# zellerlab/GECCO

Measured on AMD Instinct MI355X. Metric: genes/sec CRF decode (windowed fwd-bwd marginals + Viterbi), higher is better.
Workload: dtype f64

## Files before the change

gecco_amd/csrc/crf_scan.hpp:

```cpp
#pragma once
#include "crf_device.hpp"

namespace gecco {
namespace {

constexpr int kScanThreads = 256;

struct MapOp {
    static __device__ __forceinline__ uint32_t identity() { return 2u; }
    static __device__ __forceinline__ uint32_t combine(uint32_t a, uint32_t b) {
        return ((a >> (b & 1u)) & 1u) | (((a >> ((b >> 1) & 1u)) & 1u) << 1);
    }
};


template <int CTRL, int RM>
__device__ __forceinline__ double dpp_f64(double old, double src) {
    int lo = __builtin_amdgcn_update_dpp(__double2loint(old), __double2loint(src), CTRL, RM, 0xF, false);
    int hi = __builtin_amdgcn_update_dpp(__double2hiint(old), __double2hiint(src), CTRL, RM, 0xF, false);
    return __hiloint2double(hi, lo);
}
template <int CTRL, int RM>
__device__ __forceinline__ VE dpp_elem(const VE &old, const VE &s) {
    return VE{dpp_f64<CTRL, RM>(old.a00, s.a00), dpp_f64<CTRL, RM>(old.a01, s.a01), dpp_f64<CTRL, RM>(old.a10, s.a10),
              dpp_f64<CTRL, RM>(old.a11, s.a11), dpp_f64<CTRL, RM>(old.rs, s.rs)};
}
template <int CTRL, int RM>
__device__ __forceinline__ FE dpp_elem(const FE &old, const FE &s) {
    return FE{dpp_f64<CTRL, RM>(old.a00, s.a00), dpp_f64<CTRL, RM>(old.a01, s.a01), dpp_f64<CTRL, RM>(old.a10, s.a10),
              dpp_f64<CTRL, RM>(old.a11, s.a11), dpp_f64<CTRL, RM>(old.ex, s.ex),   dpp_f64<CTRL, RM>(old.ms, s.ms),
              dpp_f64<CTRL, RM>(old.rs, s.rs)};
}
template <int CTRL, int RM>
__device__ __forceinline__ CE dpp_elem(const CE &old, const CE &s) {
    return CE{dpp_f64<CTRL, RM>(old.a, s.a), dpp_f64<CTRL, RM>(old.L, s.L), dpp_f64<CTRL, RM>(old.H, s.H)};
}
template <int CTRL, int RM>
__device__ __forceinline__ SegE dpp_elem(const SegE &old, const SegE &s) {
    auto mv = [](uint32_t o, uint32_t v) { return uint32_t(__builtin_amdgcn_update_dpp(int(o), int(v), CTRL, RM, 0xF, false)); };
    return SegE{mv(old.map, s.map), mv(old.ng0, s.ng0), mv(old.ng1, s.ng1), mv(old.ann, s.ann)};
}
struct F4 {
    double a00, a01, a10, a11;
};
template <int CTRL, int RM>
__device__ __forceinline__ F4 dpp_elem(const F4 &old, const F4 &s) {
    return F4{dpp_f64<CTRL, RM>(old.a00, s.a00), dpp_f64<CTRL, RM>(old.a01, s.a01), dpp_f64<CTRL, RM>(old.a10, s.a10),
              dpp_f64<CTRL, RM>(old.a11, s.a11)};
}
struct U2 {
    uint32_t x, y;
};
template <int CTRL, int RM>
__device__ __forceinline__ U2 dpp_elem(const U2 &old, const U2 &s) {
    auto mv = [](uint32_t o, uint32_t v) { return uint32_t(__builtin_amdgcn_update_dpp(int(o), int(v), CTRL, RM, 0xF, false)); };
    return U2{mv(old.x, s.x), mv(old.y, s.y)};
}
struct AddOp {
    static __device__ __forceinline__ U2 identity() { return U2{0u, 0u}; }
    static __device__ __forceinline__ U2 combine(const U2 &a, const U2 &b) { return U2{a.x + b.x, a.y + b.y}; }
};
template <int CTRL, int RM>
__device__ __forceinline__ uint32_t dpp_elem(const uint32_t &old, const uint32_t &s) {
    return uint32_t(__builtin_amdgcn_update_dpp(int(old), int(s), CTRL, RM, 0xF, false));
}

template <class Op, bool REV, class E>
__device__ __forceinline__ E comb(const E &earlier_lane, const E &later_lane) {
    return REV ? Op::combine(later_lane, earlier_lane) : Op::combine(earlier_lane, later_lane);
}
template <class Op, bool REV, class E>
__device__ __forceinline__ E wave_scan_inclusive(E v) {
    const E id = Op::identity();
    v = comb<Op, REV>(dpp_elem<0x111, 0xF>(id, v), v);
    v = comb<Op, REV>(dpp_elem<0x112, 0xF>(id, v), v);
    v = comb<Op, REV>(dpp_elem<0x114, 0xF>(id, v), v);
    v = comb<Op, REV>(dpp_elem<0x118, 0xF>(id, v), v);
    v = comb<Op, REV>(dpp_elem<0x142, 0xA>(id, v), v);
    v = comb<Op, REV>(dpp_elem<0x143, 0xC>(id, v), v);
    return v;
}
template <int CTRL>
__device__ __forceinline__ double dpp_f64_z(double src) {
    int lo = __builtin_amdgcn_update_dpp(0, __double2loint(src), CTRL, 0xF, 0xF, true);
    int hi = __builtin_amdgcn_update_dpp(0, __double2hiint(src), CTRL, 0xF, 0xF, true);
    return __hiloint2double(hi, lo);
}
template <class Op>
__device__ __forceinline__ CE wave_scan_inclusive_masked(CE v) {
    const uint32_t lane = __builtin_amdgcn_mbcnt_hi(~0u, __builtin_amdgcn_mbcnt_lo(~0u, 0u));
    const uint32_t col = lane & 15u;
#define GECCO_MASKED_STEP(CTRL, COND)                                                  \
    {                                                                                  \
        CE t{dpp_f64_z<CTRL>(v.a), dpp_f64_z<CTRL>(v.L), dpp_f64_z<CTRL>(v.H)};         \
        if (COND) Op::combine_into(t, v);                                              \
    }
    GECCO_MASKED_STEP(0x111, col >= 1u)
    GECCO_MASKED_STEP(0x112, col >= 2u)
    GECCO_MASKED_STEP(0x114, col >= 4u)
    GECCO_MASKED_STEP(0x118, col >= 8u)
    GECCO_MASKED_STEP(0x142, (lane & 16u) != 0u)
    GECCO_MASKED_STEP(0x143, lane >= 32u)
#undef GECCO_MASKED_STEP
    return v;
}
template <class E>
__device__ __forceinline__ E wave_shift_up(const E &id, const E &v) {
    return dpp_elem<0x138, 0xF>(id, v);
}
template <class Op, bool REV, class E, int NTH = kScanThreads, bool MASKED = false, bool LAST_USE = false>
__device__ __forceinline__ E block_scan_exclusive(const E &mine, E *lds_totals , E *total) {
    const int lane = threadIdx.x & 63, wave = __builtin_amdgcn_readfirstlane(int(threadIdx.x >> 6));
    const E id = Op::identity();
    E incl;
    if constexpr (MASKED) {
        static_assert(!REV, "the masked scan runs in lane order");
        incl = wave_scan_inclusive_masked<Op>(mine);
    } else {
        incl = wave_scan_inclusive<Op, REV>(mine);
    }
    if (lane == 63) lds_totals[wave] = incl;
    E excl = wave_shift_up(id, incl);
    __syncthreads();
    E pre = id, all = id;
#pragma unroll
    for (int w = 0; w < NTH / 64; ++w) {
        const E t = lds_totals[w];
        if (w < wave) pre = comb<Op, REV>(pre, t);
        if (total) all = comb<Op, REV>(all, t);
    }
    if (!LAST_USE) __syncthreads();
    if (total) *total = all;
    return comb<Op, REV>(pre, excl);
}

template <class Op, int NTH = kScanThreads>
__device__ __forceinline__ uint32_t block_scan_exclusive_back(uint32_t mine, uint32_t *lds_totals , uint32_t *total,
                                                              int *vote = nullptr) {
    const int lane = threadIdx.x & 63, wave = __builtin_amdgcn_readfirstlane(int(threadIdx.x >> 6));
    const uint32_t id = Op::identity();
    const int mirror = (63 - lane) << 2;
    const uint32_t m = uint32_t(__builtin_amdgcn_ds_bpermute(mirror, int(mine)));
    const uint32_t incl = wave_scan_inclusive<Op, true>(m);
    if (lane == 63) lds_totals[wave] = incl;
    const uint32_t excl = wave_shift_up(id, incl);
    if (vote) *vote = __syncthreads_or(*vote);
    else __syncthreads();
    uint32_t pre = id, all = id;
#pragma unroll
    for (int w = NTH / 64 - 1; w >= 0; --w) {
        const uint32_t t = lds_totals[w];
        if (w > wave) pre = comb<Op, true>(pre, t);
        all = comb<Op, true>(all, t);
    }
    *total = all;
    return uint32_t(__builtin_amdgcn_ds_bpermute(mirror, int(comb<Op, true>(pre, excl))));
}

}
}
```

gecco_amd/csrc/crf_vd_short.hpp:

```cpp
#pragma once

#include "crf_device.hpp"
#include "crf_scan.hpp"

namespace gecco {
namespace {

constexpr int kT = 256;
constexpr int kGPL = kSeqGenesPerLane;
constexpr int kBlockGenes = kT * kGPL;
static_assert(kBlockGenes == kSeqBlockGenes, "host tables assume this block size");

__device__ __forceinline__ double vd_max(double a, double b) {
    double r;
    asm("v_max_f64 %0, %1, %2" : "=v"(r) : "v"(a), "v"(b));
    return r;
}
__device__ __forceinline__ double vd_min(double a, double b) {
    double r;
    asm("v_min_f64 %0, %1, %2" : "=v"(r) : "v"(a), "v"(b));
    return r;
}
__device__ __forceinline__ double vd_max_s(double a, double bound) {
    double r;
    asm("v_max_f64 %0, %1, %2" : "=v"(r) : "v"(a), "s"(bound));
    return r;
}
__device__ __forceinline__ double vd_min_s(double a, double bound) {
    double r;
    asm("v_min_f64 %0, %1, %2" : "=v"(r) : "v"(a), "s"(bound));
    return r;
}
__device__ __forceinline__ void vd_shift_in_gt(uint32_t &acc, double x, double bound) {
    asm("v_cmp_lt_f64 vcc, %2, %1\n\tv_addc_co_u32 %0, vcc, %0, %0, vcc" : "+v"(acc) : "v"(x), "s"(bound) : "vcc");
}
struct COp {
    static __device__ __forceinline__ CE identity() { return CE{0.0, -__builtin_huge_val(), __builtin_huge_val()}; }
    static __device__ __forceinline__ CE combine(const CE &a, const CE &b) {
        return CE{a.a + b.a, vd_min(vd_max(a.L + b.a, b.L), b.H), vd_min(vd_max(a.H + b.a, b.L), b.H)};
    }
    static __device__ __forceinline__ void combine_into(CE &t, CE &v) {
        asm volatile(
            "v_add_f64 %[tl], %[tl], %[a]\n\t"
            "v_add_f64 %[th], %[th], %[a]\n\t"
            "v_add_f64 %[a], %[ta], %[a]\n\t"
            "v_max_f64 %[tl], %[tl], %[L]\n\t"
            "v_max_f64 %[th], %[th], %[L]\n\t"
            "v_min_f64 %[L], %[tl], %[H]\n\t"
            "v_min_f64 %[H], %[th], %[H]"
            : [a] "+v"(v.a), [L] "+v"(v.L), [H] "+v"(v.H), [tl] "+v"(t.L), [th] "+v"(t.H)
            : [ta] "v"(t.a));
    }
};

__device__ __forceinline__ double vd_bound(const SeqArgs &A, double nnz, double n) { return nnz * A.v_wmax2 + (n + 2.0) * A.v_tmax; }
constexpr double kVdEps = 2.220446049250313e-16;
__device__ __forceinline__ double vd_margin(double r, double ulpM) { return (4.0 * r + 4.0) * ulpM; }

constexpr int kFixChunk = 1024;
struct FixStage {
    double2 st[kFixChunk];
    uint32_t bpw[kFixChunk / 16];
};
__device__ __forceinline__ void exact_states(const SeqArgs &A, int g0, int m, FixStage &fx, int first_lane) {
    const int nl = kT - first_lane, me = int(threadIdx.x) - first_lane;
    if (me < 0) return;
    for (int base = me; base < m; base += 4 * nl) {
        int lo[4], hi[4];
        double s0[4], s1[4];
        int longest = 0;
#pragma unroll
        for (int u = 0; u < 4; ++u) {
            const int i = base + u * nl;
            lo[u] = hi[u] = 0;
            if (i < m) {
                lo[u] = A.csr_gene_ptr[g0 + i];
                hi[u] = A.csr_gene_ptr[g0 + i + 1];
            }
            s0[u] = s1[u] = 0.0;
        }
#pragma unroll
        for (int u = 0; u < 4; ++u) longest = max(longest, hi[u] - lo[u]);
        for (int k = 0; k < longest; ++k) {
            int a[4];
#pragma unroll
            for (int u = 0; u < 4; ++u) a[u] = lo[u] + k < hi[u] ? A.csr_attr_id[lo[u] + k] : -1;
            double2 w[4];
#pragma unroll
            for (int u = 0; u < 4; ++u) w[u] = unsigned(a[u]) < unsigned(A.csr_n_attrs) ? A.csr_wtab01[a[u]] : make_double2(0.0, 0.0);
#pragma unroll
            for (int u = 0; u < 4; ++u) {
                s0[u] += w[u].x;
                s1[u] += w[u].y;
            }
        }
#pragma unroll
        for (int u = 0; u < 4; ++u) {
            const int i = base + u * nl;
            if (i < m) fx.st[i] = make_double2(s0[u], s1[u]);
        }
    }
}
__device__ __forceinline__ void exact_walk(const SeqArgs &A, FixStage &fx, int m, bool first, double &d0, double &d1) {
    int i = 0;
    if (first) {
        d0 = fx.st[0].x;
        d1 = fx.st[0].y;
        i = 1;
    }
    auto step = [&](const double2 s) {
        const double a0 = d0 + A.t00, b0 = d1 + A.t10;
        const double a1 = d0 + A.t01, b1 = d1 + A.t11;
        d0 = fmax(a0, b0) + s.x;
        d1 = fmax(a1, b1) + s.y;
    };
    for (; i < m && (i & 7); ++i) {
        step(fx.st[i]);
        fx.st[i] = make_double2(d0, d1);
    }
    for (; i + 8 <= m; i += 8) {
        double2 sv[8];
#pragma unroll
        for (int u = 0; u < 8; ++u) sv[u] = fx.st[i + u];
#pragma unroll
        for (int u = 0; u < 8; ++u) {
            step(sv[u]);
            fx.st[i + u] = make_double2(d0, d1);
        }
    }
    for (; i < m; ++i) {
        step(fx.st[i]);
        fx.st[i] = make_double2(d0, d1);
    }
}
__device__ __forceinline__ void exact_backpointers(const SeqArgs &A, FixStage &fx, int m, bool first, double e0, double e1) {
    for (int w = threadIdx.x; 16 * w < m; w += kT) {
        uint32_t word = 0;
        for (int i = max(16 * w, first ? 1 : 0); i < min(16 * w + 16, m); ++i) {
            const double p0 = i ? fx.st[i - 1].x : e0, p1 = i ? fx.st[i - 1].y : e1;
            const uint32_t arg0 = (p0 + A.t00) < (p1 + A.t10) ? 1u : 0u, arg1 = (p0 + A.t01) < (p1 + A.t11) ? 1u : 0u;
            word |= (arg0 | (arg1 << 1)) << (2 * (i & 15));
        }
        fx.bpw[w] = word;
    }
}
__device__ __forceinline__ uint32_t *exact_bp_words(const SeqArgs &A, int gs) { return reinterpret_cast<uint32_t *>(A.alpha) + size_t(gs); }
__device__ __forceinline__ uint32_t *exact_end_labels(const SeqArgs &A, int gs) {
    return reinterpret_cast<uint32_t *>(A.alpha) + size_t(A.n_genes) + size_t(gs);
}
__device__ __forceinline__ void exact_backtrack(const SeqArgs &A, int gs, int ge, double d0, double d1) {
    const int n = ge - gs, nw = (n + 15) / 16;
    uint32_t *bpc = exact_bp_words(A, gs), *endl = exact_end_labels(A, gs);
    auto word_map = [&](uint32_t bits, int w, uint32_t y) {
        const int hi = min(16 * w + 15, n - 1), lo = max(16 * w, 1);
        for (int t = hi; t >= lo; --t) y = (bits >> (2 * (t & 15) + y)) & 1u;
        return y;
    };
    for (int w = threadIdx.x; w < nw; w += kT) {
        const uint32_t bits = bpc[w];
        endl[w] = word_map(bits, w, 0) | (word_map(bits, w, 1) << 1);
    }
    __syncthreads();
    if (threadIdx.x == 0) {
        uint32_t y = d0 < d1 ? 1u : 0u;
        for (int w = nw - 1; w >= 0; --w) {
            const uint32_t mp = endl[w];
            endl[w] = y;
            y = (mp >> y) & 1u;
        }
    }
    __syncthreads();
    for (int w = threadIdx.x; w < nw; w += kT) {
        const uint32_t bits = bpc[w];
        uint32_t y = endl[w];
        const int hi = min(16 * w + 15, n - 1), lo = 16 * w;
        for (int t = hi; t >= lo; --t) {
            A.y[gs + t] = int8_t(y);
            if (t >= 1) y = (bits >> (2 * (t & 15) + y)) & 1u;
        }
    }
    __syncthreads();
}

__device__ __forceinline__ void exact_delta_contig(const SeqArgs &A, int gs, int ge, FixStage &fx) {
    uint32_t *bpc = exact_bp_words(A, gs);
    double d0 = 0.0, d1 = 0.0;
    for (int cb = gs; cb < ge; cb += kFixChunk) {
        const int m = min(kFixChunk, ge - cb);
        const double e0 = d0, e1 = d1;
        exact_states(A, cb, m, fx, 0);
        __syncthreads();
        if (threadIdx.x == 0) exact_walk(A, fx, m, cb == gs, d0, d1);
        __syncthreads();
        d0 = fx.st[m - 1].x;
        d1 = fx.st[m - 1].y;
        exact_backpointers(A, fx, m, cb == gs, e0, e1);
        __syncthreads();
        for (int i = threadIdx.x; i < (m + 15) / 16; i += kT) bpc[(cb - gs) / 16 + i] = fx.bpw[i];
        __syncthreads();
    }
    exact_backtrack(A, gs, ge, d0, d1);
}

constexpr double kVdPad = 1e30;

struct VdShortSmem {
    double st[kT * (kGPL + 1)];
    uint32_t mark[kBlockGenes / 32];
    int c_end;
    CE tot[kT / 64];
    uint32_t mtot[kT / 64];
};
static_assert(sizeof(VdShortSmem) <= 20480, "eight workgroups per CU");
__device__ __forceinline__ void load_short(const double *__restrict__ v, int g0, int n, VdShortSmem &stg, double (&x)[kGPL]) {
    const int base = int(threadIdx.x) * kGPL;
    const double *vp = v + g0;
#pragma unroll
    for (int k = 0; k < kGPL; ++k) x[k] = vp[max(min(base + k, n - 1), 0)];
    double *row = stg.st + threadIdx.x * (kGPL + 1);
#pragma unroll
    for (int k = 0; k < kGPL; ++k) {
        x[k] = base + k < n ? x[k] : kVdPad;
        row[k] = x[k];
    }
}

__device__ __forceinline__ uint32_t wave_or_u32(uint32_t v) {
    v |= uint32_t(__builtin_amdgcn_update_dpp(0, int(v), 0x111, 0xF, 0xF, true));
    v |= uint32_t(__builtin_amdgcn_update_dpp(0, int(v), 0x112, 0xF, 0xF, true));
    v |= uint32_t(__builtin_amdgcn_update_dpp(0, int(v), 0x114, 0xF, 0xF, true));
    v |= uint32_t(__builtin_amdgcn_update_dpp(0, int(v), 0x118, 0xF, 0xF, true));
    v |= uint32_t(__builtin_amdgcn_update_dpp(0, int(v), 0x142, 0xA, 0xF, true));
    v |= uint32_t(__builtin_amdgcn_update_dpp(0, int(v), 0x143, 0xC, 0xF, true));
    return uint32_t(__builtin_amdgcn_readlane(int(v), 63));
}

__device__ __forceinline__ void vd_short_block(const SeqArgs &A, const int blk, VdShortSmem &stg) {
    CE *lds = stg.tot;
    uint32_t *ldsm = stg.mtot;
    const int slot = threadIdx.x;
    const int g0 = __builtin_amdgcn_readfirstlane(A.cblk[blk]), n = __builtin_amdgcn_readfirstlane(A.cblk[blk + 1]) - g0;
    const uint32_t bits = A.lane_bits[blk * kT + slot];
    const uint32_t first = bits & 0xffu, last = bits >> 8;
    const uint32_t wave_bits = wave_or_u32(bits);
    double x[kGPL];
    load_short(A.dstate, g0, n, stg, x);
    const int cnt = min(kGPL, n - slot * kGPL);
    const double *row = stg.st + slot * (kGPL + 1);
    CE P = COp::identity();
#pragma unroll
    for (int k = 0; k < kGPL; ++k) {
        const double dvk = x[k];
        const bool fst = (first >> k) & 1u;
        const double c = A.v_k + dvk;
        const double l2 = vd_min_s(vd_max_s(P.L, A.v_lo), A.v_hi) + c, h2 = vd_min_s(vd_max_s(P.H, A.v_lo), A.v_hi) + c;
        P.a += c;
        P.L = l2;
        P.H = h2;
        if ((wave_bits >> k) & 1u) {
            asm volatile("" ::: "memory");
            P.L = fst ? dvk : l2;
            P.H = fst ? dvk : h2;
        }
    }
    const CE M = block_scan_exclusive<COp, false, CE, kScanThreads, true, true>(P, lds, static_cast<CE *>(nullptr));
    double ulpM = 0.0, margin = 1e-6 * fmax(1.0, fmax(fabs(A.v_lo), fabs(A.v_hi)));
    if (A.csr_gene_ptr) {
        ulpM = vd_bound(A, double(A.csr_gene_ptr[g0 + n] - A.csr_gene_ptr[g0]), double(n)) * kVdEps;
        margin = vd_margin(double(n), ulpM);
    }
    ulpM = __hiloint2double(__builtin_amdgcn_readfirstlane(__double2hiint(ulpM)), __builtin_amdgcn_readfirstlane(__double2loint(ulpM)));
    margin = __hiloint2double(__builtin_amdgcn_readfirstlane(__double2hiint(margin)), __builtin_amdgcn_readfirstlane(__double2loint(margin)));
    uint32_t maps = 0, lane_map;
    bool sensitive = false;
    {
        double Dq = M.L;
#pragma unroll
        for (int k = 0; k < kGPL; ++k) {
            const double dvk = row[k];
            const double stepped = vd_min_s(vd_max_s(Dq, A.v_lo), A.v_hi) + (A.v_k + dvk);
            Dq = stepped;
            if ((wave_bits >> k) & 1u) {
                asm volatile("" ::: "memory");
                Dq = ((first >> k) & 1u) ? dvk : stepped;
            }
            vd_shift_in_gt(maps, Dq, A.v_lo);
            vd_shift_in_gt(maps, Dq, A.v_hi);
            bool sens = fabs(Dq - A.v_hi) <= margin || fabs(Dq - A.v_lo) <= margin;
            if ((wave_bits >> (8 + k)) & 1u) {
                asm volatile("" ::: "memory");
                const bool lst = (last >> k) & 1u;
                maps = lst ? ((maps & ~3u) | (Dq > 0.0 ? 3u : 0u)) : maps;
                sens = lst ? fabs(Dq) <= margin : sens;
            }
            sensitive |= sens;
        }
    }
    auto label_map = [&]() {
        uint32_t y0 = 0u, y1 = 1u;
#pragma unroll
        for (int k = kGPL - 1; k >= 0; --k) {
            y0 = __builtin_amdgcn_ubfe(maps, uint32_t(2 * (kGPL - 1 - k)) | y0, 1u);
            y1 = __builtin_amdgcn_ubfe(maps, uint32_t(2 * (kGPL - 1 - k)) | y1, 1u);
        }
        return y0 | (y1 << 1);
    };
    const bool lane_sensitive = sensitive && A.v_exact;
    int vote = lane_sensitive ? 1 : 0;
    uint32_t mtotal;
    lane_map = label_map();
    uint32_t lab = block_scan_exclusive_back<MapOp>(lane_map, ldsm, &mtotal, &vote) & 1u;
    const bool wg_sensitive = vote != 0;
    if (wg_sensitive) {
        double Dq = M.L;
        uint64_t sat = 0;
#pragma unroll
        for (int k = 0; k < kGPL; ++k) {
            if (k < cnt) {
                const double dvk = row[k];
            Dq = ((first >> k) & 1u) ? dvk : fmin(fmax(Dq, A.v_lo), A.v_hi) + (A.v_k + dvk);
                const uint64_t c = Dq >= A.v_hi + margin ? 1u : (Dq <= A.v_lo - margin ? 2u : 0u);
                sat |= c << (8 * k);
            }
        }
        *reinterpret_cast<uint64_t *>(&stg.st[slot * (kGPL + 1) + kGPL]) = sat;
        __syncthreads();
    } else {
        sensitive = false;
    }
    bool lane_flagged = false;
    if (sensitive && cnt > 0) {
        double D = 0.0;
        int r = 0;
        auto certain = [&](double x) { return x >= A.v_hi + margin || x <= A.v_lo - margin; };
        if (!(first & 1u)) {
            const int t0 = slot * kGPL;
            int p = t0 - 1;
            auto dval = [&](int t) { return stg.st[(t / kGPL) * (kGPL + 1) + t % kGPL]; };
            for (;; --p) {
                if (A.flags[g0 + p] & 1u) {
                    D = dval(p);
                    r = 0;
                    break;
                }
                const uint32_t c = reinterpret_cast<const uint8_t *>(&stg.st[((p - 1) / kGPL) * (kGPL + 1) + kGPL])[(p - 1) % kGPL];
                if (c) {
                    D = (c == 1u ? A.v_hi : A.v_lo) + (A.v_k + dval(p));
                    r = 1;
                    break;
                }
            }
            for (int t = p + 1; t < t0; ++t) {
                r = certain(D) ? 1 : r + 1;
                D = fmin(fmax(D, A.v_lo), A.v_hi) + (A.v_k + dval(t));
            }
        }
        maps = 0;
#pragma unroll
        for (int k = 0; k < kGPL; ++k) {
            if (k < cnt) {
                const double dvk = row[k];
                const bool fst = (first >> k) & 1u;
                r = fst ? 0 : (certain(D) ? 1 : r + 1);
                D = fst ? dvk : fmin(fmax(D, A.v_lo), A.v_hi) + (A.v_k + dvk);
                const bool lst = (last >> k) & 1u;
                const double thi = lst ? 0.0 : A.v_hi, tlo = lst ? 0.0 : A.v_lo;
                maps |= ((D > thi ? 1u : 0u) | (D > tlo ? 2u : 0u)) << (2 * (kGPL - 1 - k));
                const double mr = vd_margin(double(r), ulpM);
                lane_flagged |= fabs(D - thi) <= mr || fabs(D - tlo) <= mr;
            }
        }
        if (A.vd_stats) {
            atomicAdd(A.vd_stats + 0, 1u);
            if (lane_flagged) atomicAdd(A.vd_stats + 1, 1u);
        }
    }
    bool wg_flagged = false;
    if (wg_sensitive) {
        wg_flagged = __syncthreads_or(lane_flagged ? 1 : 0);
        lane_map = label_map();
        lab = block_scan_exclusive_back<MapOp>(lane_map, ldsm, &mtotal) & 1u;
    }
    uint64_t packed = 0;
#pragma unroll
    for (int k = kGPL - 1; k >= 0; --k) {
        lab = __builtin_amdgcn_ubfe(maps, uint32_t(2 * (kGPL - 1 - k)) | lab, 1u);
        packed |= uint64_t(lab) << (8 * k);
    }
    {
        struct __attribute__((packed)) Bytes8 {
            uint64_t v;
        };
        int8_t *yp = A.y + g0 + slot * kGPL;
        if (cnt >= kGPL) {
            reinterpret_cast<Bytes8 *>(yp)->v = packed;
        } else {
            for (int k = 0; k < cnt; ++k) yp[k] = int8_t(packed >> (8 * k));
        }
    }
    if (wg_flagged && A.csr_gene_ptr) {
        uint32_t *mark = stg.mark;
        int *c_end = &stg.c_end;
        __syncthreads();
        if (slot < kBlockGenes / 32) mark[slot] = 0;
        __syncthreads();
        if (lane_flagged) {
            int prev = -1;
            for (int k = 0; k < cnt; ++k) {
                int t = slot * kGPL + k;
                while (!(A.flags[g0 + t] & 1u)) --t;
                if (t != prev) atomicOr(&mark[t >> 5], 1u << (t & 31));
                prev = t;
            }
        }
        __syncthreads();
        FixStage &st2 = *reinterpret_cast<FixStage *>(stg.st);
        static_assert(sizeof(stg.st) >= sizeof(FixStage), "exact pass: LDS for one chunk of state scores");
        for (int wi = 0; wi < kBlockGenes / 32; ++wi) {
            uint32_t bits = mark[wi];
            while (bits) {
                const int cs = wi * 32 + __builtin_ctz(bits);
                bits &= bits - 1;
                if (slot == 0) *c_end = n;
                __syncthreads();
                for (int i = cs + slot; i < n; i += kT)
                    if (A.flags[g0 + i] & 2u) {
                        atomicMin(c_end, i + 1);
                        break;
                    }
                __syncthreads();
                const int ce = *c_end;
                __syncthreads();
                if (slot == 0 && A.vd_stats) {
                    atomicAdd(A.vd_stats + 2, 1u);
                    atomicAdd(A.vd_stats + 3, uint32_t(ce - cs));
                }
                exact_delta_contig(A, g0 + cs, g0 + ce, st2);
            }
        }
    }
}

}
}
```

Measured before the change: 73.35 billion.

## Replace clamp scan with short saturation-based propagation and LDS ballot votes

Replaces the full block-wide masked scan of clamp-affine elements with a short local propagation that starts from lanes whose clamp interval has collapsed (L==H). Each lane inherits its neighbour's value for up to a few DPP steps, and the full scan runs only when some wave cannot resolve its inputs that way. It also replaces __syncthreads_or with wave ballots posted to LDS, adds a fast unclamped load path for full waves, and computes sensitivity through one min-abs distance. This cuts scan work and barrier cost in the common saturated case, but adds a fallback branch, extra LDS state and more intricate correctness conditions.

```diff
diff --git a/gecco_amd/csrc/crf_scan.hpp b/gecco_amd/csrc/crf_scan.hpp
--- a/gecco_amd/csrc/crf_scan.hpp
+++ b/gecco_amd/csrc/crf_scan.hpp
@@ -134,9 +134,23 @@
     return comb<Op, REV>(pre, excl);
 }
 
+template <int NTH = kScanThreads>
+__device__ __forceinline__ void block_or_post(bool mine, uint32_t *lds_votes ) {
+    const int wave = __builtin_amdgcn_readfirstlane(int(threadIdx.x >> 6));
+    const uint32_t any = __builtin_amdgcn_ballot_w64(mine) != 0 ? 1u : 0u;
+    if ((threadIdx.x & 63) == 63) lds_votes[wave] = any;
+}
+template <int NTH = kScanThreads>
+__device__ __forceinline__ bool block_or_read(const uint32_t *lds_votes ) {
+    uint32_t any = 0;
+#pragma unroll
+    for (int w = 0; w < NTH / 64; ++w) any |= lds_votes[w];
+    return __builtin_amdgcn_readfirstlane(int(any)) != 0;
+}
+
 template <class Op, int NTH = kScanThreads>
 __device__ __forceinline__ uint32_t block_scan_exclusive_back(uint32_t mine, uint32_t *lds_totals , uint32_t *total,
-                                                              int *vote = nullptr) {
+                                                              int *vote = nullptr, uint32_t *lds_votes  = nullptr) {
     const int lane = threadIdx.x & 63, wave = __builtin_amdgcn_readfirstlane(int(threadIdx.x >> 6));
     const uint32_t id = Op::identity();
     const int mirror = (63 - lane) << 2;
@@ -144,8 +158,9 @@
     const uint32_t incl = wave_scan_inclusive<Op, true>(m);
     if (lane == 63) lds_totals[wave] = incl;
     const uint32_t excl = wave_shift_up(id, incl);
-    if (vote) *vote = __syncthreads_or(*vote);
-    else __syncthreads();
+    if (vote) block_or_post<NTH>(*vote != 0, lds_votes);
+    __syncthreads();
+    if (vote) *vote = block_or_read<NTH>(lds_votes) ? 1 : 0;
     uint32_t pre = id, all = id;
 #pragma unroll
     for (int w = NTH / 64 - 1; w >= 0; --w) {
diff --git a/gecco_amd/csrc/crf_vd_short.hpp b/gecco_amd/csrc/crf_vd_short.hpp
--- a/gecco_amd/csrc/crf_vd_short.hpp
+++ b/gecco_amd/csrc/crf_vd_short.hpp
@@ -19,6 +19,11 @@
 __device__ __forceinline__ double vd_min(double a, double b) {
     double r;
     asm("v_min_f64 %0, %1, %2" : "=v"(r) : "v"(a), "v"(b));
+    return r;
+}
+__device__ __forceinline__ double vd_min_abs(double a, double b) {
+    double r;
+    asm("v_min_f64 %0, |%1|, |%2|" : "=v"(r) : "v"(a), "v"(b));
     return r;
 }
 __device__ __forceinline__ double vd_max_s(double a, double bound) {
@@ -210,14 +215,25 @@
     int c_end;
     CE tot[kT / 64];
     uint32_t mtot[kT / 64];
+    double pv[kT / 64];
+    uint32_t pbad[kT / 64];
+    uint32_t vote[kT / 64];
 };
 static_assert(sizeof(VdShortSmem) <= 20480, "eight workgroups per CU");
 __device__ __forceinline__ void load_short(const double *__restrict__ v, int g0, int n, VdShortSmem &stg, double (&x)[kGPL]) {
     const int base = int(threadIdx.x) * kGPL;
     const double *vp = v + g0;
+    double *row = stg.st + threadIdx.x * (kGPL + 1);
+    const int wave_end = (__builtin_amdgcn_readfirstlane(int(threadIdx.x >> 6)) + 1) * 64 * kGPL;
+    if (wave_end <= n) {
+#pragma unroll
+        for (int k = 0; k < kGPL; ++k) x[k] = vp[base + k];
+#pragma unroll
+        for (int k = 0; k < kGPL; ++k) row[k] = x[k];
+        return;
+    }
 #pragma unroll
     for (int k = 0; k < kGPL; ++k) x[k] = vp[max(min(base + k, n - 1), 0)];
-    double *row = stg.st + threadIdx.x * (kGPL + 1);
 #pragma unroll
     for (int k = 0; k < kGPL; ++k) {
         x[k] = base + k < n ? x[k] : kVdPad;
@@ -233,6 +249,20 @@
     v |= uint32_t(__builtin_amdgcn_update_dpp(0, int(v), 0x142, 0xA, 0xF, true));
     v |= uint32_t(__builtin_amdgcn_update_dpp(0, int(v), 0x143, 0xC, 0xF, true));
     return uint32_t(__builtin_amdgcn_readlane(int(v), 63));
+}
+
+constexpr int kVdRun = 6;
+__device__ __forceinline__ void vd_apply(const CE &P, double in, double &v) {
+    asm volatile("v_add_f64 %0, %1, %2\n\tv_max_f64 %0, %0, %3\n\tv_min_f64 %0, %0, %4" : "+v"(v) : "v"(in), "v"(P.a), "v"(P.L), "v"(P.H));
+}
+__device__ __forceinline__ void vd_propagate(const CE &P, double &v, uint64_t &known) {
+    for (int it = 0; it < kVdRun; ++it) {
+        const uint64_t todo = (known << 1) & ~known;
+        if (!todo) break;
+        const double in = dpp_f64_z<0x138>(v);
+        if (__builtin_amdgcn_inverse_ballot_w64(todo)) vd_apply(P, in, v);
+        known |= todo;
+    }
 }
 
 __device__ __forceinline__ void vd_short_block(const SeqArgs &A, const int blk, VdShortSmem &stg) {
@@ -263,7 +293,29 @@
             P.H = fst ? dvk : h2;
         }
     }
-    const CE M = block_scan_exclusive<COp, false, CE, kScanThreads, true, true>(P, lds, static_cast<CE *>(nullptr));
+    double Din;
+    {
+        const int wave = __builtin_amdgcn_readfirstlane(int(threadIdx.x >> 6));
+        double v = P.L;
+        uint64_t known = __builtin_amdgcn_ballot_w64(P.L == P.H);
+        vd_propagate(P, v, known);
+        const bool wave_bad = (known | (known - 1)) != ~uint64_t(0) || !(known & (wave ? (uint64_t(2) << kVdRun) - 1 : uint64_t(1)));
+        if ((threadIdx.x & 63) == 63) stg.pv[wave] = v;
+        block_or_post(wave_bad, stg.pbad);
+        __syncthreads();
+        if (block_or_read(stg.pbad)) {
+            const CE M = block_scan_exclusive<COp, false, CE, kScanThreads, true, true>(P, lds, static_cast<CE *>(nullptr));
+            Din = M.L;
+        } else {
+            const double carry = stg.pv[wave ? wave - 1 : 0];
+            if (!(known & 1u)) {
+                if ((threadIdx.x & 63) == 0) vd_apply(P, carry, v);
+                known |= 1u;
+                vd_propagate(P, v, known);
+            }
+            Din = dpp_f64<0x138, 0xF>(carry, v);
+        }
+    }
     double ulpM = 0.0, margin = 1e-6 * fmax(1.0, fmax(fabs(A.v_lo), fabs(A.v_hi)));
     if (A.csr_gene_ptr) {
         ulpM = vd_bound(A, double(A.csr_gene_ptr[g0 + n] - A.csr_gene_ptr[g0]), double(n)) * kVdEps;
@@ -274,7 +326,7 @@
     uint32_t maps = 0, lane_map;
     bool sensitive = false;
     {
-        double Dq = M.L;
+        double Dq = Din, nearest = __builtin_huge_val();
 #pragma unroll
         for (int k = 0; k < kGPL; ++k) {
             const double dvk = row[k];
@@ -286,15 +338,16 @@
             }
             vd_shift_in_gt(maps, Dq, A.v_lo);
             vd_shift_in_gt(maps, Dq, A.v_hi);
-            bool sens = fabs(Dq - A.v_hi) <= margin || fabs(Dq - A.v_lo) <= margin;
+            double dist = vd_min_abs(Dq - A.v_hi, Dq - A.v_lo);
             if ((wave_bits >> (8 + k)) & 1u) {
                 asm volatile("" ::: "memory");
                 const bool lst = (last >> k) & 1u;
                 maps = lst ? ((maps & ~3u) | (Dq > 0.0 ? 3u : 0u)) : maps;
-                sens = lst ? fabs(Dq) <= margin : sens;
-            }
-            sensitive |= sens;
-        }
+                dist = lst ? fabs(Dq) : dist;
+            }
+            nearest = vd_min(nearest, dist);
+        }
+        sensitive = nearest <= margin;
     }
     auto label_map = [&]() {
         uint32_t y0 = 0u, y1 = 1u;
@@ -309,10 +362,10 @@
     int vote = lane_sensitive ? 1 : 0;
     uint32_t mtotal;
     lane_map = label_map();
-    uint32_t lab = block_scan_exclusive_back<MapOp>(lane_map, ldsm, &mtotal, &vote) & 1u;
+    uint32_t lab = block_scan_exclusive_back<MapOp>(lane_map, ldsm, &mtotal, &vote, stg.vote) & 1u;
     const bool wg_sensitive = vote != 0;
     if (wg_sensitive) {
-        double Dq = M.L;
+        double Dq = Din;
         uint64_t sat = 0;
 #pragma unroll
         for (int k = 0; k < kGPL; ++k) {
@@ -377,7 +430,9 @@
     }
     bool wg_flagged = false;
     if (wg_sensitive) {
-        wg_flagged = __syncthreads_or(lane_flagged ? 1 : 0);
+        block_or_post(lane_flagged, stg.vote);
+        __syncthreads();
+        wg_flagged = block_or_read(stg.vote);
         lane_map = label_map();
         lab = block_scan_exclusive_back<MapOp>(lane_map, ldsm, &mtotal) & 1u;
     }
```

After: 76.12 billion, median of 6. 1.04x the previous value.
